# microsoft/mgl

Hardware: AMD Instinct MI355X
Metric: GCUPS (+ aligned reads/s) for 150 bp short-read batch (higher is better)
Workload: dtype int16; 1 GPU; BASELINE.json configs[1]: 10000000 Illumina-style 150 bp reads x 256-base reference windows, affine-gap SW, full matrix, GATK params (200,-150,260,11), SOFTCLIP, scores+offset+CIGAR for every pair; pairs_total=10000000, pairs_per_gpu=10000000, target_len=256, query_len=150, input=ascii, parallelism=1 GPU, steps_in_flight=1

## Files before the change

### mgl_amd/csrc/sw_capi.cpp

```cpp
#include "../../include/mgl_sw.h"

#include <hip/hip_runtime.h>

#include <algorithm>
#include <chrono>
#include <cstdint>
#include <cstdio>
#include <functional>
#include <future>
#include <cstring>
#include <mutex>
#include <string>
#include <vector>

#include "sw_ctx_access.h"
#include "sw_device.h"

using namespace mgl_sw_dev;

static_assert(sizeof(mgl_sw_score) == sizeof(Score), "mgl_sw_score layout");

namespace {

constexpr int64_t kDefaultWorkspace = 4ll << 30;
// ... 828 lines not shown
                HIP_TRY(ctx, hipEventSynchronize(ctx->srt_done[k & 3]));
                RegroupArgs ra;
                (void)sort_chunk(first, count, (int)(k & 3), &ra);
                rg.d_t_start = ra.t_start;
                rg.d_q_start = ra.q_start;
                rg.d_dest = ra.dest;
                rg.d_t_len = ra.t_len;
                rg.d_q_len = ra.q_len;
                rg.n_grouped = ctx->pin_total[2 * (k & 3)];
                rg.n_lane = ctx->pin_total[2 * (k & 3) + 1];
                if (rg.n_grouped < 0 || rg.n_grouped > count || (rg.n_grouped & 7) || rg.n_lane < 0 || rg.n_lane > rg.n_grouped || (rg.n_lane & 127))
                    return fail(ctx, MGL_SW_ERR_DEVICE, "sorting a chunk by geometry failed");
                if (!hooks) {
                    const int src = sort_until(k + 2);
                    if (src != MGL_SW_OK) return src;
                }
                sort_more = hooks != nullptr;
            }
            const SeqSet ts{tset.data, rg.d_t_start, rg.d_t_len, max_tl, tset.packed2}, qs{qset.data, rg.d_q_start, rg.d_q_len, max_ql, qset.packed2};
            const int64_t ng = rg.n_grouped;
            const char *const lgm = getenv("MGL_SW_DEBUG_LANE_GROUP_MIN");
            const int64_t lane_group_min = lgm ? (int64_t)atoll(lgm) : kLaneGroupMinPairs;
            const int64_t nl = lane_group && rg.n_lane >= std::max<int64_t>(lane_group_min, 128) ? rg.n_lane : 0;
            uint32_t *const tb16 = tb_base + (size_t)std::min<int64_t>(nl / 128, lane_slots) * (size_t)lane_group_stride;
            lane_pairs_last = nl;
            if (nl > 0) parts.push_back(Part{true, false, 0, nl, ts, qs, tb_base, lane_group_stride, rec_base, rg.d_dest, 32, 4, max_ql, false});
            if (P.group_regions) {
                uint32_t *const area16 = tb_base + (size_t)lane_slots * (size_t)lane_group_stride, *const area32 = area16 + (size_t)(P.left_area / 2 / 4);
                const int64_t cap16 = std::max<int64_t>(8, P.left_area / 2 / P.left_pair16 / 8 * 8), cap32 = std::max<int64_t>(4, P.left_area / 2 / P.left_pair32 / 4 * 4);
                for (int64_t f = nl; f < ng; f += cap16)
                    parts.push_back(Part{false, true, f, std::min(cap16, ng - f), ts, qs, area16, stride_words, rec_base + f, rg.d_dest, 16, wpb16, sps_for(max_ql), f + cap16 < ng});
                for (int64_t f = ng; f < count; f += cap32)
                    parts.push_back(Part{false, false, f, std::min(cap32, count - f), ts, qs, area32, stride32_words, rec_base + f, rg.d_dest, 16,
                                         pick_waves_per_block(sps32, 16), sps32, f + cap32 < count});
            } else {
                if (ng > nl) parts.push_back(Part{false, true, nl, ng - nl, ts, qs, tb16, stride_words, rec_base + nl, rg.d_dest, 16, wpb16, sps_for(max_ql), false});
                if (count > ng)
                    parts.push_back(Part{false, false, ng, count - ng, ts, qs, tb16 + (size_t)((ng - nl) / 2) * (size_t)stride_words, stride32_words,
                                         rec_base + ng, rg.d_dest, 16, pick_waves_per_block(sps32, 16), sps32, false});
            }
        }
        const int n_parts = (int)parts.size();
        const char *const sre = getenv("MGL_SW_DEBUG_SIDE_RESERVE");
        const int64_t side_reserve = sre ? atoll(sre) : kSideReserve;
        const bool side = P.group_regions && side_reserve > 0;
        std::vector<DpArgs> das((size_t)n_parts);
        std::vector<TbArgs> tas((size_t)n_parts);
        int64_t n_blocks = 0;
        for (int i = 0; i < n_parts; ++i) {
            const Part &pt = parts[i];
            DpArgs &da = das[i];
            da.t = pt.t;
            da.q = pt.q;
            da.first = pt.first;
            da.count = pt.count;
            da.match = match;
            da.mismatch = mismatch;
            da.gopen = gopen;
            da.gext = gext;
            da.strategy = strategy;
            da.sps_cap = pt.sps_cap;
            da.uni_tl = max_tl;
            da.uni_ql = max_ql;
            da.tb = pt.tb;
            da.tb_stride_words = pt.stride;
            da.rec = pt.rec;
            da.scratch = pt.lane ? static_cast<unsigned char *>(ctx->bnd[h].p) : (use_scratch || coop_waves || strip16) ? static_cast<unsigned char *>(ctx->scratch.p) : nullptr;
            da.diag = nullptr;
            da.matrix = d_matrix;
            da.code = d_code;
            da.matrix_lds_offset = 0;
            da.score_only = score_only ? 1 : 0;
            da.grouped = pt.lane && auto_group ? 1 : 0;
            da.strip_k = strip16 ? strip_k : 0;
            da.strip_passes = strip16 ? strip_passes : 0;
            {
                const char *const sce = getenv("MGL_SW_DEBUG_STRIP_CODES");
                da.strip_codes = strip16 && strip_k > 0 && !(sce && atoi(sce) == 0) && strip16_lds_bytes_codes(max_ql, strip_waves) <= 64 * 1024 ? 1 : 0;
            }
            da.fold_k = P.fold.k;
            da.fold_bm = P.fold.bm;
            da.fold_bx = P.fold.bx;
            da.lane_slots = 0;
            da.tile_ctr = nullptr;
            da.grid_fault = nullptr;
            da.gate = nullptr;
            da.gate_dev = nullptr;
            da.gate_failed = nullptr;
            da.gate_timeout_ticks = 0;
            if (pt.lane && (lane_ck || da.grouped)) {
                da.lane_slots = (int)std::min<int64_t>(lane_slots - (side && n_parts > 1 ? std::min<int64_t>(side_reserve, lane_slots / 2) : 0), (pt.count + 127) / 128);
                if (ctx->cur_gate && !hooks) {
                    da.gate = ctx->cur_gate;
                    da.gate_dev = ctx->cur_gate_dev;
                    da.gate_failed = reinterpret_cast<int32_t *>(const_cast<int64_t *>(ctx->cur_gate) + 1);
                    da.gate_timeout_ticks = 100000000u;
                    if (const char *const gte = getenv("MGL_SW_DEBUG_GATE_TIMEOUT_TICKS")) da.gate_timeout_ticks = (unsigned)atoll(gte);
                }
                if ((pt.count + 127) / 128 > da.lane_slots) {
                    da.tile_ctr = static_cast<unsigned *>(ctx->tile_ctr.p) + (size_t)(ctx->tile_seq++ % kTileCounters) * kTileCounterWords;
                    void *fault_dev = nullptr;
                    HIP_TRY(ctx, hipHostGetDevicePointer(&fault_dev, ctx->pin_fault, 0));
                    da.grid_fault = static_cast<int32_t *>(fault_dev);
                }
            }
            const int per_block = pt.lane ? pt.wpb * 128 : pt.packed ? pt.wpb * 8 : strip16 ? 1 : pt.wpb * (64 / pt.rows);
            if (i == 0) n_blocks = da.lane_slots > 0 ? da.lane_slots : (pt.count + per_block - 1) / per_block;
            if (ctx->profiling == 2 && i == 0) {
                HIP_TRY(ctx, ctx->diag.reserve((size_t)n_blocks * 16));
                da.diag = static_cast<unsigned long long *>(ctx->diag.p);
            }
            TbArgs &ta = tas[i];
            ta.t = pt.t;
            ta.q = pt.q;
            ta.first = pt.first;
            ta.count = pt.count;
            ta.strategy = strategy;
            ta.tb = pt.tb;
            ta.tb_stride_words = pt.stride;
            ta.packed16 = pt.lane ? 2 : pt.packed ? 1 : strip16 ? (strip_k ? 6 : 4) : coop16 ? 3 : 0;
            ta.match = match;
            ta.mismatch = mismatch;
            ta.gopen = gopen;
            ta.gext = gext;
            ta.strip_rows = pt.rows;
            ta.strip_k = strip16 ? strip_k : 0;
            ta.rows_per_stripe = pt.rows;
            ta.uni_ql = max_ql;
            ta.rec = pt.rec;
            ta.offset = d_offset;
            ta.score = d_score;
            ta.cigar = d_cigar;
            ta.cigar_stride = cigar_stride;
            ta.binary_cigar = binary_cigar ? 1 : 0;
            ta.cigar_len = d_cigar_len;
            ta.status = d_status;
            ta.status_any = hooks ? hooks->d_status_any : ctx->direct_status_any;
            ta.dest = pt.dest;
            const char *const colds = getenv("MGL_SW_DEBUG_COALESCED_OUT");
            ta.coalesced_out = pt.lane && (lane_ck || da.grouped) && !(colds && atoi(colds) == 0) && lane_ck_coalesced_ok(ta) ? 1 : 0;
        }

        hipEvent_t pe[4] = {nullptr, nullptr, nullptr, nullptr};
        if (ctx->profiling) {
            while ((int)ctx->pool.size() < ctx->pool_used + 4) {
                hipEvent_t e = nullptr;
                HIP_TRY(ctx, hipEventCreate(&e));
                ctx->pool.push_back(e);
            }
            for (int i = 0; i < 4; ++i) pe[i] = ctx->pool[(size_t)ctx->pool_used + i];
            ctx->pool_used += 4;
            ctx->diag_blocks = n_blocks;
        }
        hipStream_t tb_stream = overlap ? ctx->aux : fs;
        if ((overlap || side) && tb_pending[h]) HIP_TRY(ctx, hipStreamWaitEvent(fs, ctx->tb_done[h], 0));
        if (side && n_parts > 1) {
            if (k == 0 && ctx->ws_idle_set) HIP_TRY(ctx, hipStreamWaitEvent(ctx->aux, ctx->ws_idle, 0));
            if (side_grid_pending[h]) HIP_TRY(ctx, hipStreamWaitEvent(ctx->aux, ctx->fill_done[h], 0));
            for (int i = 0; i < n_parts; ++i) {
                const Part &pt = parts[i];
                if (pt.lane) continue;
                HIP_TRY(ctx, pt.packed ? launch_dp16(das[i], pt.wpb, ctx->aux) : launch_dp(das[i], pt.wpb, pt.rows, ctx->aux));
                HIP_TRY(ctx, launch_traceback(tas[i], ctx->aux));
            }
            HIP_TRY(ctx, hipEventRecord(ctx->tb_done[h], ctx->aux));
            tb_pending[h] = true;
// ... 1967 lines not shown
```

### mgl_amd/csrc/sw_device.h

```cpp
#ifndef MGL_SW_DEVICE_H
#define MGL_SW_DEVICE_H

#include <hip/hip_runtime.h>
#include <stddef.h>
#include <stdint.h>

namespace mgl_sw_dev {

constexpr int NEG_INF = -0x40000000;
constexpr int OS_SOFTCLIP = 1, OS_INDEL = 2, OS_LEAD_ID = 4, OS_IGNORE = 8;
constexpr int ERR_CIGAR_OVERFLOW = 2;
constexpr int ERR_DEVICE = 4;
constexpr int MATRIX_DIM = 32;

struct Score {
    int32_t mqe, mqe_t, max, max_t, max_q, seg_length;
};

struct DpRecord {
    int32_t mqe, mqe_t, max, max_t, max_q, seg;
    int32_t g_tail;
    int32_t sps;
};

struct SeqSet {
    const uint8_t *data;
    const int64_t *off;
    const int32_t *len;
    int uni_len;
    int packed2;
    __host__ __device__ inline int length(int64_t p) const
    {
        if (len) return len[p];
        return packed2 ? uni_len : (int)(off[p + 1] - off[p]);
    }
    __device__ inline int at(int64_t start, int k) const
    {
        const int64_t pos = start + k;
        if (packed2) return (data[pos >> 2] >> (2 * (int)(pos & 3))) & 3;
        return data[pos];
    }
};

struct DpArgs {
    SeqSet t, q;
    int64_t first;
    int64_t count;
    int match, mismatch, gopen, gext, strategy;
    int sps_cap;
    int uni_tl, uni_ql;
    uint32_t *tb;
    int64_t tb_stride_words;
    DpRecord *rec;
    unsigned char *scratch;
    unsigned long long *diag;
    const int8_t *matrix;
    const uint8_t *code;
    int matrix_lds_offset;
    int score_only;
    int grouped;
    int strip_k;
    int strip_passes;
    int strip_codes;
    int lane_slots;
    unsigned *tile_ctr;
    int32_t *grid_fault;
    const int64_t *gate;
    int64_t *gate_dev;
    int32_t *gate_failed;
    unsigned gate_timeout_ticks;
    const int32_t *tile_order;
    const int64_t *slot_off;
    int fold_k, fold_bm, fold_bx;
};

struct TbArgs {
    SeqSet t, q;
    int64_t first, count;
    int strategy;
    const uint32_t *tb;
    int64_t tb_stride_words;
    int packed16;
    int rows_per_stripe;
    int uni_ql;
    const DpRecord *rec;
    int32_t *offset;
    Score *score;
    char *cigar;
    int cigar_stride;
    int binary_cigar;
    int32_t *cigar_len;
    int32_t *status;
    int32_t *status_any;
    int match, mismatch, gopen, gext;
    int strip_rows, strip_k;
    const int64_t *dest;
    int coalesced_out;
};

__host__ __device__ inline int sps_for_rows(int ql, int rows) { return (ql + rows + 3) & ~3; }
__host__ __device__ inline int sps_for(int ql) { return sps_for_rows(ql, 16); }
__host__ __device__ inline int stripes_for(int tl) { return (tl + 15) >> 4; }
__host__ __device__ inline int dp_ring_entries(int sps_cap, int rows) { return sps_cap + rows + 4; }
__host__ __device__ inline int dp_qcopy_bytes(int sps_cap, int rows) { return sps_cap + rows + 16; }
__host__ __device__ inline int64_t tb_words_for(int tl, int sps, int rows)
{
    return ((((int64_t)(tl + rows - 1) / rows) * sps + 31) >> 5) * rows * 4;
}

__host__ __device__ inline int dp16_base(int tl, int ql, int match, int gext)
{
    return 32767 - match * (tl < ql ? tl : ql) - gext * (tl + ql);
}
__host__ __device__ inline int dp16_period(int ql) { return (ql + 1 + 3) & ~3; }
__host__ __device__ inline int dp16_chained_stripes(int tl, int ql)
{
    if (dp16_period(ql) < 32) return 0;
    const int n = stripes_for(tl);
    return (tl & 15) == 0 ? n : n - 1;
}
__host__ __device__ inline int64_t dp16_total_steps(int tl, int ql)
{
    const int n = stripes_for(tl), nc = dp16_chained_stripes(tl, ql);
    return (nc ? (int64_t)nc * dp16_period(ql) + 16 : 0) + (int64_t)(n - nc) * sps_for(ql);
}
__host__ __device__ inline int64_t tb_words16_for(int tl, int ql) { return ((dp16_total_steps(tl, ql) + 7) >> 3) * 32; }
__host__ __device__ inline int64_t tb_words16_bound(int tl, int ql) { return (((int64_t)stripes_for(tl) * sps_for(ql) + 16 + 7) >> 3) * 32; }

__host__ __device__ inline int lane_strips(int tl, int rows) { return (tl + rows - 1) / rows; }
__host__ __device__ inline int64_t lane_tb_words(int tl, int ql, int rows) { return (int64_t)lane_strips(tl, rows) * ql * (rows / 16) * 64 * 4; }
__host__ __device__ inline int64_t lane_bnd_entries(int ql) { return (int64_t)(ql + 1) * 64; }
__host__ __device__ inline int64_t lane_scratch_bytes(int tl, int ql, int rows)
{
    return lane_bnd_entries(ql) * 8 + ((int64_t)((ql + 3) / 4) + (int64_t)lane_strips(tl, rows) * (rows / 4)) * 2 * 64 * 4;
}

__host__ __device__ inline int coop_sps_for(int ql) { return (ql + 64 + 31) & ~31; }
__host__ __device__ inline int coop16_sps_for(int ql) { return (ql + 129 + 31) & ~31; }
__host__ __device__ inline int64_t tb_words_coop16(int tl, int ql) { return (int64_t)((tl + 127) >> 7) * (coop16_sps_for(ql) >> 4) * 64 * 4; }
__host__ __device__ inline int coop_query_bytes(int sps_cap) { return (sps_cap + 192 + 15) & ~15; }
__host__ __device__ inline int coop_wrap_cols(int sps_cap) { return sps_cap + 192; }

constexpr int LANE_CK_COLS = 32;
__host__ __device__ inline int lane_ck_blocks(int ql) { return (ql + LANE_CK_COLS - 1) / LANE_CK_COLS; }
__host__ __device__ inline int64_t lane_ck_words(int tl, int ql)
{
    const int64_t strips = lane_strips(tl, 32);
    return ((strips + 1) * (ql + 1) * 2 + strips * ql * 2 + strips * (lane_ck_blocks(ql) - 1) * 64 + (int64_t)LANE_CK_COLS * 4) * 64;
}
__host__ __device__ inline int64_t lane_ck_scratch_bytes(int tl, int ql) { return ((int64_t)((ql + 3) / 4) + (int64_t)lane_strips(tl, 32) * 8) * 2 * 64 * 4; }
constexpr int LANE_CK_OUT_STRIDE_MAX = 64;
constexpr int LANE_CK_OUT_LDS_BYTES = 128 * (LANE_CK_OUT_STRIDE_MAX + 24 + 12);
__host__ inline bool lane_ck_coalesced_ok(const TbArgs &a)
{
    auto al = [](const void *p) { return (reinterpret_cast<uintptr_t>(p) & 15u) == 0; };
    return !a.dest && !a.binary_cigar && a.cigar_stride >= 4 && a.cigar_stride <= LANE_CK_OUT_STRIDE_MAX && (a.cigar_stride & 3) == 0 && al(a.cigar) && al(a.offset) &&
           al(a.score) && al(a.cigar_len) && al(a.status) && (a.first & 127) == 0;
}
constexpr int LANE_CK_WAVES_PER_CU = 8;
__host__ __device__ inline int64_t lane_ck_region_bytes(int tl, int ql) { return lane_ck_words(tl, ql) * 4 + lane_ck_scratch_bytes(tl, ql); }
__host__ __device__ inline int64_t lane_ck_slots(int64_t pairs, int n_cus, int64_t bytes, int tl, int ql)
{
    const int64_t tiles = (pairs + 127) / 128, chip = (int64_t)n_cus * LANE_CK_WAVES_PER_CU, fit = bytes / lane_ck_region_bytes(tl, ql);
    const int64_t s = tiles < chip ? tiles : chip;
    return s < fit ? s : fit;
}

int64_t dp_group_bytes(int sps_cap, int rows);
int dp_lds_bytes(int sps_cap, int waves_per_block, int rows);
int dp16_lds_bytes(int sps, int waves_per_block);
bool dp16_range_ok(int tl, int ql, int match, int mismatch, int gopen, int gext, int strategy);
struct DiagFold {
    int k, bm, bx;
};
__host__ __device__ inline int ctz16(unsigned x)
{
    int s = 0;
    while (!(x & 1u)) x >>= 1, ++s;
    return s;
}
__host__ __device__ inline unsigned inv_odd16(unsigned o)
{
    unsigned x = o;
    for (int i = 0; i < 3; ++i) x *= 2u - o * x;
    return x & 0xffffu;
}
__host__ __device__ inline int fold_byte(unsigned k, unsigned v)
{
    const int s = ctz16(k);
    if (v & ((1u << s) - 1u)) return -1;
    const unsigned b = ((v >> s) * inv_odd16(k >> s)) & ((0x10000u >> s) - 1u);
    return b <= 255u ? (int)b : -1;
}
__host__ __device__ inline DiagFold diag_fold(int match, int mismatch, int gext)
{
    const unsigned a = (unsigned)(match + 2 * gext) & 0xffffu, x = (unsigned)(mismatch + 2 * gext) & 0xffffu;
    const unsigned p = a ? a : x;
    DiagFold d{0, 0, 0};
    if (!p) return DiagFold{1, 0, 0};
    for (unsigned b = 1; b < 256u; ++b) {
        const int u = ctz16(b);
        if (p & ((1u << u) - 1u)) continue;
        const unsigned period = 0x10000u >> u;
        for (unsigned k = ((p >> u) * inv_odd16(b >> u)) & (period - 1u); k < 0x10000u && (d.k == 0 || k < (unsigned)d.k); k += period) {
            if (k == 0) continue;
            const int bm = fold_byte(k, a), bx = fold_byte(k, x);
            if (bm >= 0 && bx >= 0) {
                d = DiagFold{(int)k, bm, bx};
                break;
            }
        }
    }
    return d;
}
hipError_t launch_dp16(const DpArgs &a, int waves_per_block, hipStream_t stream);
bool lane16_supported(const SeqSet &t, const SeqSet &q);
bool lane16_ck_supported(const SeqSet &t, const SeqSet &q);
struct TbArgs;
hipError_t launch_dp16_lane(const DpArgs &a, const TbArgs &walk, int rows, hipStream_t stream);
bool lane16_matrix_params_ok(int smin, int smax, int gopen, int gext);
int lane16_matrix_lds_bytes(int max_tl);
hipError_t launch_dp16_lane_matrix(const DpArgs &a, const TbArgs &walk, hipStream_t stream);
__host__ __device__ inline int64_t lane16_matrix_tb_bytes(int tl, int ql, bool score_only) { return score_only ? 0 : lane_tb_words(tl, ql, 32) * 4; }
__host__ __device__ inline int64_t lane16_matrix_region_bytes(int tl, int ql, bool score_only) { return (lane16_matrix_tb_bytes(tl, ql, score_only) + lane_scratch_bytes(tl, ql, 32) + 255) / 256 * 256; }
hipError_t launch_tile_geometry(const SeqSet &t, const SeqSet &q, int64_t first, int64_t count, int32_t *out, hipStream_t stream);
hipError_t launch_dp16_lane_ck(const DpArgs &a, const TbArgs &walk, hipStream_t stream);
hipError_t launch_dp(const DpArgs &a, int waves_per_block, int rows, hipStream_t stream);
int coop_lds_bytes(int sps_cap, int waves_per_block);
hipError_t launch_dp_coop(const DpArgs &a, int waves_per_block, hipStream_t stream);
bool coop16_possible(int match, int mismatch, int gopen, int gext);
bool coop16_worthwhile(int match, int mismatch, int gopen, int gext);
int coop16_lds_bytes(int sps_cap, int waves_per_block);
constexpr int STRIP_CPS = 4;
__host__ __device__ inline int strip16_groups(int ql) { return (ql + STRIP_CPS - 1) / STRIP_CPS; }
__host__ __device__ inline int strip16_steps(int ql, int waves) { return strip16_groups(ql) + 2 * 64 * waves - 1; }
// ... 94 lines not shown
```

### mgl_amd/csrc/sw_dp16_lane_ck.hip

```cpp
#include <hip/hip_runtime.h>
#include <stdint.h>
#include <stdio.h>
#include <stdlib.h>
#include <string.h>

#include "sw_device.h"
#include "sw_lane_cell.h"
#include "sw_traceback.h"

#ifndef MGL_CK_ABLATE
#define MGL_CK_ABLATE 0
#endif
#if (MGL_CK_ABLATE != 0 || defined(MGL_CK_PHASES) || defined(MGL_CK_TRACE)) && !defined(MGL_VARIANT_BUILD)
#error "MGL_CK_ABLATE / MGL_CK_PHASES are measurement builds (scripts/build_variant.sh defines MGL_VARIANT_BUILD): never the shipped library"
#endif

#ifdef MGL_CK_PHASES
__device__ unsigned long long mgl_ck_phase_ticks[16];
#define CK_PHASE(k)                                                                                    \
    do {                                                                                               \
        const unsigned long long now_ = __builtin_amdgcn_s_memtime();                                  \
        if (lane == 0) atomicAdd(&mgl_ck_phase_ticks[k], now_ - phase_t0);                             \
        phase_t0 = __builtin_amdgcn_s_memtime();                                                       \
    } while (0)
// ... 489 lines not shown
    {
        const unsigned ia = (unsigned)((((sA >> 1) * (g.nb - 1) + max(bA - 1, 0)) * 64 + (sA & 1) * 2 * RB) * 64) + wm.lane;
        const unsigned ib = (unsigned)((((sB >> 1) * (g.nb - 1) + max(bB - 1, 0)) * 64 + (sB & 1) * 2 * RB) * 64) + wm.lane;
        unsigned v[2 * RB];
#pragma unroll
        for (int x = 0; x < 2 * RB; ++x) v[x] = 0u;
        if (needA && bA > 0) {
#pragma unroll
            for (int x = 0; x < 2 * RB; ++x) v[x] = WaveMem::at32<unsigned>(wm.cku, 4u * (ia + (unsigned)(x * 64)));
        }
#pragma unroll
        for (int r = 0; r < RB; ++r) {
            const int rowA = sA * RB + r + 1;
            const int fa_ = border(rowA, g.gopen, g.gext, g.indel) + rowA * g.gext + g.base;
            h[r] = bA > 0 ? v[2 * r] : (unsigned)fa_;
            f[r] = bA > 0 ? v[2 * r + 1] : (unsigned)(fa_ - (g.gopen - g.gext));
        }
#pragma unroll
        for (int x = 0; x < 2 * RB; ++x) v[x] = 0u;
        if (needB && bB > 0) {
#pragma unroll
            for (int x = 0; x < 2 * RB; ++x) v[x] = WaveMem::at32<unsigned>(wm.cku, 4u * (ib + (unsigned)(x * 64)));
        }
#pragma unroll
        for (int r = 0; r < RB; ++r) {
            const int rowB = sB * RB + r + 1;
            const int fb_ = border(rowB, g.gopen, g.gext, g.indel) + rowB * g.gext + g.base;
            const unsigned hb = bB > 0 ? v[2 * r] : (unsigned)fb_ << 16, gb = bB > 0 ? v[2 * r + 1] : (unsigned)(fb_ - (g.gopen - g.gext)) << 16;
            h[r] = lo_hi(h[r], hb);
            f[r] = lo_hi(f[r], gb);
        }
    }
    unsigned hd;
    {
        unsigned a0 = 0u, b0 = 0u;
        if (needA) a0 = wm.row16(sA, g.ql, CK * bA).x;
        if (needB) b0 = wm.row16(sB, g.ql, CK * bB).x;
        if (sA & 1) {
            const int row = sA * RB;
            const int v = border(row, g.gopen, g.gext, g.indel) + row * g.gext + g.base;
            a0 = bA > 0 ? a0 : (unsigned)v;
        }
        if (sB & 1) {
            const int row = sB * RB;
            const int v = border(row, g.gopen, g.gext, g.indel) + row * g.gext + g.base;
            b0 = bB > 0 ? b0 : (unsigned)v << 16;
        }
        hd = lo_hi(a0, b0);
    }
    const int qmax = ((g.ql + 3) >> 2) - 1;
#pragma unroll 1
    for (int gg = 0; gg < groups; ++gg) {
        uint2 va[8], vb[8];
#pragma unroll
        for (int u = 0; u < 8; ++u) va[u] = vb[u] = make_uint2(0u, 0u);
        if (needA) {
#pragma unroll
            for (int u = 0; u < 8; ++u) va[u] = wm.row16(sA, g.ql, min(CK * bA + 8 * gg + u + 1, g.ql));
        }
        if (needB) {
#pragma unroll
            for (int u = 0; u < 8; ++u) vb[u] = wm.row16(sB, g.ql, min(CK * bB + 8 * gg + u + 1, g.ql));
        }
        unsigned qa[2], qb[2];
#pragma unroll
        for (int u = 0; u < 2; ++u) {
            qa[u] = wm.qblock(min(bA * (CK / 4) + 2 * gg + u, qmax), 0);
            qb[u] = wm.qblock(min(bB * (CK / 4) + 2 * gg + u, qmax), 1);
        }
#pragma unroll
        for (int u = 0; u < 8; ++u) {
            unsigned e = lo_hi(va[u].y, vb[u].y);
            uint4 *const out = wm.blk + (size_t)(8 * gg + u) * 64;
            if (CODES)
                column<RB, false, false, CODES>(h, f, t, code_table((qa[u >> 2] >> (8 * (u & 3))) & 0xffu, c.bm, c.bx), hd, e, c, out, nullptr,
                                                code_table((qb[u >> 2] >> (8 * (u & 3))) & 0xffu, c.bm, c.bx));
            else
                column<RB, false, false, false>(h, f, t, __builtin_amdgcn_perm(qb[u >> 2], qa[u >> 2], 0x0c040c00u + 0x00010001u * (u & 3)), hd, e, c, out);
            hd = lo_hi(va[u].x, vb[u].x);
        }
    }
}

typedef uint32_t dwords4 __attribute__((ext_vector_type(4), aligned(4)));
__device__ __forceinline__ void seq_words4(const SeqWords &s, const int k0, unsigned (&w)[4])
{
    if (k0 + 3 <= s.kmax) {
        const dwords4 v = *reinterpret_cast<const dwords4 *>(s.base + k0);
        w[0] = v.x;
        w[1] = v.y;
        w[2] = v.z;
        w[3] = v.w;
    } else {
#pragma unroll
        for (int u = 0; u < 4; ++u) w[u] = s.word(k0 + u);
    }
}
template <bool CODES, bool QUERY>
__device__ __forceinline__ unsigned stage_ascii(const uint8_t *seqA, const uint8_t *seqB, const int len, const int nblocks, unsigned *dst)
{
    SeqWords sa, sb;
    sa.init(seqA, len);
    sb.init(seqB, len);
    unsigned bad = 0;
    for (int cb = 0; cb < nblocks; cb += 16) {
        unsigned wa[20], wb[20];
#pragma unroll
        for (int u = 0; u < 4; ++u) {
            unsigned xa[4], xb[4];
            seq_words4(sa, cb + 4 * u, xa);
            seq_words4(sb, cb + 4 * u, xb);
#pragma unroll
            for (int x = 0; x < 4; ++x) {
                wa[4 * u + x] = xa[x];
                wb[4 * u + x] = xb[x];
            }
        }
        wa[16] = sa.word(cb + 16);
        wb[16] = sb.word(cb + 16);
#pragma unroll
        for (int u = 0; u < 16; ++u) {
            if (cb + u < nblocks) {
                unsigned va = __builtin_amdgcn_alignbyte(wa[u + 1], wa[u], sa.shift), vb = __builtin_amdgcn_alignbyte(wb[u + 1], wb[u], sb.shift);
                if (CODES) {
                    unsigned da, db;
                    va = ascii_codes(va, da);
                    vb = ascii_codes(vb, db);
                    if (QUERY) {
                        const unsigned na = nonzero_bytes(da), nb = nonzero_bytes(db);
                        va = ((va << 3) & ~((na >> 2) - (na >> 7))) | (na >> 2);
                        vb = ((vb << 3) & ~((nb >> 2) - (nb >> 7))) | (nb >> 2);
                    } else {
                        const int nv = len - 4 * (cb + u);
                        const unsigned keep = nv >= 4 ? 0xffffffffu : nv <= 0 ? 0u : (1u << (8 * nv)) - 1u;
                        bad |= (da | db) & keep;
                    }
                }
                dst[(size_t)(2 * (cb + u)) * 64] = va;
                dst[(size_t)(2 * (cb + u) + 1) * 64] = vb;
            }
        }
    }
    return bad;
}

struct Seq2Words {
    const uint32_t *base;
    unsigned shift;
    int kmax;
    __device__ __forceinline__ void init(const uint8_t *data, int64_t start, int len)
    {
        const uintptr_t a = reinterpret_cast<uintptr_t>(data) + (uintptr_t)(start >> 2), e = reinterpret_cast<uintptr_t>(data) + (uintptr_t)((start + len - 1) >> 2);
        base = reinterpret_cast<const uint32_t *>(a & ~(uintptr_t)3);
        shift = (unsigned)(a & 3) * 8u + 2u * (unsigned)(start & 3);
        kmax = (int)(((e & ~(uintptr_t)3) - (a & ~(uintptr_t)3)) >> 2);
    }
    __device__ __forceinline__ unsigned word(int k) const { return base[k < kmax ? k : kmax]; }
};
template <bool QUERY>
__device__ __forceinline__ void stage_2bit(const uint8_t *data, const int64_t startA, const int64_t startB, const int len, const int nblocks, unsigned *dst)
{
    Seq2Words sa, sb;
    sa.init(data, startA, len);
    sb.init(data, startB, len);
    for (int cb = 0; cb < nblocks; cb += 16) {
        unsigned wa[5], wb[5];
#pragma unroll
        for (int u = 0; u < 5; ++u) {
            wa[u] = sa.word((cb >> 2) + u);
            wb[u] = sb.word((cb >> 2) + u);
        }
#pragma unroll
        for (int u = 0; u < 4; ++u) {
            const unsigned va = __builtin_amdgcn_alignbit(wa[u + 1], wa[u], sa.shift), vb = __builtin_amdgcn_alignbit(wb[u + 1], wb[u], sb.shift);
#pragma unroll
            for (int x = 0; x < 4; ++x) {
                const int blk = cb + 4 * u + x;
                if (blk < nblocks) {
                    const unsigned ca = spread_2bit((va >> (8 * x)) & 0xffu), cb2 = spread_2bit((vb >> (8 * x)) & 0xffu);
                    dst[(size_t)(2 * blk) * 64] = QUERY ? ca << 3 : ca;
                    dst[(size_t)(2 * blk + 1) * 64] = QUERY ? cb2 << 3 : cb2;
                }
            }
        }
    }
}

__device__ __forceinline__ void lds_to_global(void *dst, const unsigned char *src, const int bytes, const int lane)
{
    const int whole = bytes & ~15;
    for (int k = lane * 16; k < whole; k += 1024) *reinterpret_cast<uint4 *>(static_cast<unsigned char *>(dst) + k) = *reinterpret_cast<const uint4 *>(src + k);
    for (int k = whole + lane * 4; k < bytes; k += 256) *reinterpret_cast<unsigned *>(static_cast<unsigned char *>(dst) + k) = *reinterpret_cast<const unsigned *>(src + k);
}

template <bool VIA_LDS, bool FOLD>
__device__ __forceinline__ void sw_dp16_lane_ck_tile(const DpArgs &a, const TbArgs &walk_in, const int64_t gw, const int64_t slot, const int lane, unsigned char *out_lds, const bool first)
{
    const int64_t n_ls = (a.count + 1) >> 1;
#ifdef MGL_CK_PHASES
    unsigned long long phase_t0 = __builtin_amdgcn_s_memtime();
#endif
    const int64_t ls = gw * 64 + lane;
    const bool lvalid = ls < n_ls;
    const int64_t slotA = lvalid ? 2 * ls : a.count - 1;
    const bool validB = lvalid && (2 * ls + 1 < a.count);
    const int64_t slotB = validB ? 2 * ls + 1 : slotA;

    const bool grouped = a.grouped != 0;
    const int tl = grouped ? __builtin_amdgcn_readfirstlane(a.t.length(a.first + gw * 128)) : a.uni_tl;
    const int ql = grouped ? __builtin_amdgcn_readfirstlane(a.q.length(a.first + gw * 128)) : a.uni_ql;
    const int match = a.match, gopen = a.gopen, gext = a.gext;
    const bool indel = (a.strategy & (OS_INDEL | OS_LEAD_ID)) != 0;
    const int base = dp16_base(tl, ql, match, gext);
    LaneConsts c;
    c.delta = pack2(a.mismatch - match, a.mismatch - match);
    c.one = pack2(1, 1);
    c.o_e = pack2(gopen - gext, gopen - gext);
    c.k2 = pack2(match + 2 * gext, match + 2 * gext);
    asm volatile("" : "+v"(c.delta), "+v"(c.one), "+v"(c.o_e), "+v"(c.k2));
#pragma unroll
    for (int u = 0; u < 4; ++u) {
        c.k12[u] = 0x02020202u << (2 * u);
        c.k34[u] = 0x01010101u << (2 * u);
        asm volatile("" : "+s"(c.k12[u]), "+s"(c.k34[u]));
    }
    c.kf = pack2(a.fold_k, a.fold_k);
    c.bm = FOLD ? (unsigned)a.fold_bm : 0u;
    c.bx = FOLD ? (unsigned)a.fold_bx : 1u;
    if (FOLD) asm volatile("" : "+s"(c.kf));
    constexpr int CM = FOLD ? CMP_FOLD : CMP_CODES;

    const int strips = lane_strips(tl, R), nb = lane_ck_blocks(ql);
    unsigned *const qst = reinterpret_cast<unsigned *>(a.scratch + (size_t)slot * (size_t)lane_ck_scratch_bytes(a.uni_tl, a.uni_ql)) + lane;
    unsigned *const tst = qst + (size_t)((ql + 3) >> 2) * 128;
    WaveMem wm;
    {
        uint2 *const region = reinterpret_cast<uint2 *>(a.tb + (size_t)slot * (size_t)a.tb_stride_words);
        wm.bnd = region + lane;
        wm.mid = wm.bnd + (size_t)(strips + 1) * (ql + 1) * 64;
        wm.ck = reinterpret_cast<unsigned *>(region + ((size_t)(strips + 1) * (ql + 1) + (size_t)strips * ql) * 64) + lane;
        wm.blk = reinterpret_cast<uint4 *>(reinterpret_cast<unsigned *>(region) + ((size_t)(strips + 1) * (ql + 1) * 2 + (size_t)strips * ql * 2 + (size_t)strips * (nb - 1) * 64) * 64) + lane;
        wm.rows = region;
        wm.mid_off = (unsigned)((strips + 1) * (ql + 1) * 64);
        wm.cku = reinterpret_cast<const unsigned *>(region + ((size_t)(strips + 1) * (ql + 1) + (size_t)strips * ql) * 64);
        wm.blku = reinterpret_cast<const uint32_t *>(region) + ((size_t)(strips + 1) * (ql + 1) * 2 + (size_t)strips * ql * 2 + (size_t)strips * (nb - 1) * 64) * 64;
        wm.seq = reinterpret_cast<const unsigned *>(a.scratch + (size_t)slot * (size_t)lane_ck_scratch_bytes(a.uni_tl, a.uni_ql));
        wm.t_off = (unsigned)(((ql + 3) >> 2) * 128);
        wm.lane = (unsigned)lane;
    }
    bool codes;
    {
        const int64_t pA = a.first + slotA, pB = a.first + slotB;
        const int qblocks = (ql + 3) >> 2, tblocks = strips * (R / 4);
        if (a.t.packed2) {
            stage_2bit<false>(a.t.data, a.t.off[pA], a.t.off[pB], tl, tblocks, tst);
            stage_2bit<true>(a.q.data, a.q.off[pA], a.q.off[pB], ql, qblocks, qst);
            codes = true;
        } else {
            const unsigned bad = stage_ascii<true, false>(a.t.data + a.t.off[pA], a.t.data + a.t.off[pB], tl, tblocks, tst);
            codes = __builtin_amdgcn_ballot_w64(bad != 0u) == 0;
            if (codes) {
                stage_ascii<true, true>(a.q.data + a.q.off[pA], a.q.data + a.q.off[pB], ql, qblocks, qst);
            } else {
                stage_ascii<false, false>(a.t.data + a.t.off[pA], a.t.data + a.t.off[pB], tl, tblocks, tst);
                stage_ascii<false, true>(a.q.data + a.q.off[pA], a.q.data + a.q.off[pB], ql, qblocks, qst);
            }
        }
        if (grouped || first) {
            for (int j = 0; j <= ql; ++j) {
                const int hb0 = border(j, gopen, gext, indel) + j * gext + base;
                const unsigned hp = pack2(hb0, hb0);
                wm.bnd[(size_t)j * 64] = make_uint2(hp, pk_sub(hp, c.o_e));
            }
            for (int k = 1; k <= strips; ++k) {
                const int hb0 = border(k * R, gopen, gext, indel) + k * R * gext + base;
                wm.bnd[(size_t)k * (ql + 1) * 64] = make_uint2(pack2(hb0, hb0), 0u);
            }
        }
    }
// ... 75 lines not shown
        if (half ? validB : lvalid) a.rec[half ? slotB : slotA] = r;
    }

    CK_PHASE(2);
    const int64_t pA = a.first + slotA, pB = a.first + slotB;
    constexpr bool via_lds = VIA_LDS;
    TbArgs walk = walk_in;
    unsigned char *const l_score = out_lds + 128 * LANE_CK_OUT_STRIDE_MAX, *const l_off = l_score + 128 * 24, *const l_len = l_off + 512, *const l_status = l_len + 512;
    if (via_lds) {
        walk.cigar = reinterpret_cast<char *>(out_lds);
        walk.score = walk_in.score ? reinterpret_cast<Score *>(l_score) : nullptr;
        walk.offset = reinterpret_cast<int32_t *>(l_off);
        walk.cigar_len = walk_in.cigar_len ? reinterpret_cast<int32_t *>(l_len) : nullptr;
        walk.status = walk_in.status ? reinterpret_cast<int32_t *>(l_status) : nullptr;
    }
    const int64_t oA = via_lds ? 2 * lane : walk.dest ? walk.dest[pA] : pA, oB = via_lds ? 2 * lane + 1 : walk.dest ? walk.dest[pB] : pB;
    PathWalk wa, wb;
    wa.start(walk, rec[0], oA, tl, ql, lvalid, cornerA);
    wb.start(walk, rec[1], oB, tl, ql, validB, cornerB);
    BlockGeom geom;
    geom.ql = ql;
    geom.nb = nb;
    geom.match = match;
    geom.mismatch = a.mismatch;
    geom.gopen = gopen;
    geom.gext = gext;
    geom.base = base;
    geom.indel = indel;
    geom.codes = codes;
    const bool by_score = !(MGL_CK_ABLATE & 8);
    const int tblocks = strips * (R / 4), qblocks = (ql + 3) >> 2;
    while (!(MGL_CK_ABLATE & 1) && __builtin_amdgcn_ballot_w64(!wa.done || !wb.done) != 0) {
        if (by_score) {
            for (;;) {
                unsigned ta[17], qa[17], tb[17], qb[17], ga[PathWalk::VB], gb[PathWalk::VB];
                if (wa.can_verify()) {
                    wa.win64_load(wm, 0, tblocks, qblocks, ta, qa);
                    wa.grid_load(wm, ql, ga);
                }
                if (wb.can_verify()) {
                    wb.win64_load(wm, 1, tblocks, qblocks, tb, qb);
                    wb.grid_load(wm, ql, gb);
                }
                const bool ma = wa.verify_apply(ta, qa, ga, 0, geom), mb = wb.verify_apply(tb, qb, gb, 1, geom);
#ifdef MGL_CK_PHASES
                if (lane == 0) atomicAdd(&mgl_ck_phase_ticks[12], 1ull);
#endif
                if (!__builtin_amdgcn_ballot_w64(ma || mb)) break;
            }
            {
                const int ea = wa.edge_len(), eb = wb.edge_len();
                if (__builtin_amdgcn_ballot_w64((ea | eb) != 0)) {
                    unsigned ta[5], qa[5], tb[5], qb[5], ha = 0u, hb = 0u;
                    if (ea) {
                        wa.win_load(wm, 0, tblocks, qblocks, ta, qa);
                        ha = wa.edge_load(wm, nb, ea);
                    }
                    if (eb) {
                        wb.win_load(wm, 1, tblocks, qblocks, tb, qb);
                        hb = wb.edge_load(wm, nb, eb);
                    }
                    const bool xa = wa.edge_apply(ha, ta, qa, ea, 0, geom), xb = wb.edge_apply(hb, tb, qb, eb, 1, geom);
#ifdef MGL_CK_PHASES
                    const unsigned long long took_ = __popcll(__builtin_amdgcn_ballot_w64(xa)) + __popcll(__builtin_amdgcn_ballot_w64(xb));
                    const unsigned long long tried_ = __popcll(__builtin_amdgcn_ballot_w64(ea != 0)) + __popcll(__builtin_amdgcn_ballot_w64(eb != 0));
                    if (lane == 0) {
                        atomicAdd(&mgl_ck_phase_ticks[10], took_);
                        atomicAdd(&mgl_ck_phase_ticks[11], tried_ - took_);
                    }
#else
                    (void)xa;
                    (void)xb;
#endif
                }
            }
            CK_PHASE(3);
            if (__builtin_amdgcn_ballot_w64(!wa.done || !wb.done) == 0) break;
        }
        const int kA = max(wa.pi - 1, 0) >> 4, bA = max(wa.pj - 1, 0) / CK, kB = max(wb.pi - 1, 0) >> 4, bB = max(wb.pj - 1, 0) / CK;
        int reach = max(!wa.done ? (max(wa.pj - 1, 0) % CK) + 1 : 0, !wb.done ? (max(wb.pj - 1, 0) % CK) + 1 : 0);
#pragma unroll
        for (int m = 32; m >= 1; m >>= 1) reach = max(reach, __shfl_xor(reach, m));
        const int groups = __builtin_amdgcn_readfirstlane((reach + 7) >> 3);
        if (codes)
            ck_block<CM>(kA, bA, kB, bB, !wa.done, !wb.done, geom, wm, c, groups);
        else
            ck_block<CMP_BYTES>(kA, bA, kB, bB, !wa.done, !wb.done, geom, wm, c, groups);
        asm volatile("s_waitcnt vmcnt(0)" ::: "memory");
        CK_PHASE(4);
#ifdef MGL_CK_PHASES
        if (lane == 0) atomicAdd(&mgl_ck_phase_ticks[8], 1ull);
#endif
        for (;;) {
            const bool la = wa.can_load(kA, bA), lb = wb.can_load(kB, bB);
            unsigned fa[PathWalk::LOOK], fb[PathWalk::LOOK], ta[5], qa[5], tb[5], qb[5];
            if (la) {
                wa.load(wm, fa);
                if (wa.mode == 0) wa.win_load(wm, 0, tblocks, qblocks, ta, qa);
            }
            if (lb) {
                wb.load(wm, fb);
                if (wb.mode == 0) wb.win_load(wm, 1, tblocks, qblocks, tb, qb);
            }
            const bool ga = wa.apply(fa, ta, qa, 0, kA, bA, geom), gb = wb.apply(fb, tb, qb, 1, kB, bB, geom);
            if (!__builtin_amdgcn_ballot_w64(ga || gb)) break;
        }
        wa.stuck = wb.stuck = false;
        CK_PHASE(5);
    }
    CK_PHASE(6);
    if (lvalid) wa.finish(walk, a.rec + slotA, oA);
    if (validB) wb.finish(walk, a.rec + slotB, oB);
    if (via_lds) {
        __builtin_amdgcn_fence(__ATOMIC_RELEASE, "workgroup");
        __builtin_amdgcn_wave_barrier();
        __builtin_amdgcn_fence(__ATOMIC_ACQUIRE, "workgroup");
        const int64_t p0 = a.first + gw * 128;
        const int np = (int)min((int64_t)128, a.count - gw * 128);
        lds_to_global(walk_in.cigar + (size_t)p0 * walk_in.cigar_stride, out_lds, np * walk_in.cigar_stride, lane);
        if (walk_in.score) lds_to_global(walk_in.score + p0, l_score, np * 24, lane);
        lds_to_global(walk_in.offset + p0, l_off, np * 4, lane);
        if (walk_in.cigar_len) lds_to_global(walk_in.cigar_len + p0, l_len, np * 4, lane);
        if (walk_in.status) lds_to_global(walk_in.status + p0, l_status, np * 4, lane);
        __builtin_amdgcn_wave_barrier();
    }
    CK_PHASE(7);
#ifdef MGL_CK_PHASES
    if (lane == 0) atomicAdd(&mgl_ck_phase_ticks[9], 1ull);
#endif
}

}

template <bool VIA_LDS, bool FOLD>
__device__ __forceinline__ void lane_ck_grid(const DpArgs &a, const TbArgs &walk, unsigned char *out_lds)
{
    const int lane = threadIdx.x & 63;
    const int64_t tiles = (((a.count + 1) >> 1) + 63) >> 6, slots = gridDim.x, slot = blockIdx.x;
    unsigned long long diag_t0 = 0, diag_w0 = 0;
    if (a.diag) {
        diag_t0 = __builtin_amdgcn_s_memtime();
        diag_w0 = __builtin_amdgcn_s_memrealtime();
    }
    int64_t arrived = a.gate ? 0 : INT64_MAX;
    unsigned long long *const ctr = reinterpret_cast<unsigned long long *>(a.tile_ctr);
    for (int64_t tile = slot; tile < tiles;) {
        if (arrived < a.first + min(a.count, (tile + 2) * 128)) {
            const int64_t need = a.first + min(a.count, (tile + 2) * 128);
            int lo = 0, hi = 0, flags = 0;
            if (lane == 0) {
                unsigned long long since = __builtin_amdgcn_s_memrealtime();
                long long last = arrived, seen;
                for (;;) {
                    seen = (long long)__hip_atomic_load(reinterpret_cast<const unsigned long long *>(a.gate_dev), __ATOMIC_RELAXED, __HIP_MEMORY_SCOPE_AGENT);
                    if (seen >= need || seen < 0) break;
                    const unsigned long long now = __builtin_amdgcn_s_memrealtime();
                    const unsigned long long polled = __hip_atomic_load(reinterpret_cast<const unsigned long long *>(a.gate_dev) + 1, __ATOMIC_RELAXED, __HIP_MEMORY_SCOPE_AGENT);
                    if (now - polled >= 100ull) {
                        unsigned long long expect = polled;
                        if (__hip_atomic_compare_exchange_strong(reinterpret_cast<unsigned long long *>(a.gate_dev) + 1, &expect, now, __ATOMIC_RELAXED, __ATOMIC_RELAXED, __HIP_MEMORY_SCOPE_AGENT)) {
                            const long long v = (long long)__hip_atomic_load(reinterpret_cast<const unsigned long long *>(a.gate), __ATOMIC_RELAXED, __HIP_MEMORY_SCOPE_SYSTEM);
                            if (v < 0)
                                __hip_atomic_store(reinterpret_cast<long long *>(a.gate_dev), v, __ATOMIC_RELAXED, __HIP_MEMORY_SCOPE_AGENT);
                            else
                                __hip_atomic_fetch_max(reinterpret_cast<long long *>(a.gate_dev), v, __ATOMIC_RELAXED, __HIP_MEMORY_SCOPE_AGENT);
                            seen = v;
                            if (seen >= need || seen < 0) break;
                        }
                    }
                    if (seen != last) {
                        last = seen;
                        since = now;
                    } else if (now - since > (unsigned long long)a.gate_timeout_ticks) {
                        flags = 1;
                        break;
                    }
                    __builtin_amdgcn_s_sleep(32);
                }
                lo = (int)(unsigned)(unsigned long long)seen;
                hi = (int)(unsigned)((unsigned long long)seen >> 32);
            }
            lo = __builtin_amdgcn_readfirstlane(lo);
            hi = __builtin_amdgcn_readfirstlane(hi);
            flags = __builtin_amdgcn_readfirstlane(flags);
            arrived = (int64_t)((unsigned long long)(unsigned)lo | (unsigned long long)(unsigned)hi << 32);
            if (flags & 1) {
                if (lane == 0) __hip_atomic_store(a.gate_failed, 1, __ATOMIC_RELAXED, __HIP_MEMORY_SCOPE_SYSTEM);
                break;
            }
            if (arrived < 0) break;
#ifndef MGL_CK_NO_GATE_FENCE
            __builtin_amdgcn_fence(__ATOMIC_ACQUIRE, "agent");
#endif
        }
#ifdef MGL_CK_TRACE
        const unsigned long long t0 = __builtin_amdgcn_s_memrealtime();
#endif
        sw_dp16_lane_ck_tile<VIA_LDS, FOLD>(a, walk, tile, slot, lane, out_lds, tile == slot);
#ifdef MGL_CK_TRACE
        if (lane == 0 && tile < (1 << 17)) {
            unsigned hw;
            asm volatile("s_getreg_b32 %0, hwreg(HW_REG_HW_ID)" : "=s"(hw));
            unsigned xcc;
            asm volatile("s_getreg_b32 %0, hwreg(HW_REG_XCC_ID)" : "=s"(xcc));
            mgl_ck_trace[4 * tile + 0] = (unsigned long long)slot;
            mgl_ck_trace[4 * tile + 1] = (unsigned long long)hw | (unsigned long long)(xcc & 15u) << 32;
            mgl_ck_trace[4 * tile + 2] = t0;
            mgl_ck_trace[4 * tile + 3] = __builtin_amdgcn_s_memrealtime();
        }
#endif
        if (tiles <= slots) break;
        unsigned next = 0;
        if (lane == 0) {
            next = (unsigned)__hip_atomic_fetch_add(ctr, 1ull, __ATOMIC_RELAXED, __HIP_MEMORY_SCOPE_AGENT);
            if (next >= (unsigned)tiles && a.grid_fault) __hip_atomic_store(a.grid_fault, 1, __ATOMIC_RELAXED, __HIP_MEMORY_SCOPE_SYSTEM);
        }
        tile = slots + (int64_t)(unsigned)__builtin_amdgcn_readfirstlane((int)next);
    }
    if (tiles > slots && lane == 0) {
        const unsigned out = (unsigned)(__hip_atomic_fetch_add(ctr, 1ull << 32, __ATOMIC_RELAXED, __HIP_MEMORY_SCOPE_AGENT) >> 32);
        if (out == (unsigned)slots - 1u) {
            __hip_atomic_store(ctr, 0ull, __ATOMIC_RELAXED, __HIP_MEMORY_SCOPE_AGENT);
        } else if (out >= (unsigned)slots && a.grid_fault) {
            __hip_atomic_store(a.grid_fault, 1, __ATOMIC_RELAXED, __HIP_MEMORY_SCOPE_SYSTEM);
        }
    }
    if (a.diag && lane == 0) {
        a.diag[2 * slot] = __builtin_amdgcn_s_memtime() - diag_t0;
        a.diag[2 * slot + 1] = __builtin_amdgcn_s_memrealtime() - diag_w0;
    }
}

__global__ __launch_bounds__(64, 2) void sw_dp16_lane_ck_kernel(const DpArgs a, const TbArgs walk)
{
    __shared__ __attribute__((aligned(16))) unsigned char out_lds[LANE_CK_OUT_LDS_BYTES];
    lane_ck_grid<true, false>(a, walk, out_lds);
}

__global__ __launch_bounds__(64, 2) void sw_dp16_lane_ck_scatter_kernel(const DpArgs a, const TbArgs walk) { lane_ck_grid<false, false>(a, walk, nullptr); }

__global__ __launch_bounds__(64, 2) void sw_dp16_lane_ck_kernel_fold(const DpArgs a, const TbArgs walk)
{
    __shared__ __attribute__((aligned(16))) unsigned char out_lds[LANE_CK_OUT_LDS_BYTES];
    lane_ck_grid<true, true>(a, walk, out_lds);
}
__global__ __launch_bounds__(64, 2) void sw_dp16_lane_ck_scatter_kernel_fold(const DpArgs a, const TbArgs walk) { lane_ck_grid<false, true>(a, walk, nullptr); }

bool lane16_ck_supported(const SeqSet &t, const SeqSet &q) { return (t.packed2 != 0) == (q.packed2 != 0); }

hipError_t launch_dp16_lane_ck(const DpArgs &a, const TbArgs &walk, hipStream_t stream)
{
    const int64_t tiles = ((a.count + 1) / 2 + 63) / 64;
    if (a.lane_slots < 1 || (tiles > a.lane_slots && !a.tile_ctr)) return hipErrorInvalidValue;
    const dim3 grid((unsigned)(tiles < a.lane_slots ? tiles : a.lane_slots)), block(64);
    if (walk.coalesced_out)
        hipLaunchKernelGGL(a.fold_k ? sw_dp16_lane_ck_kernel_fold : sw_dp16_lane_ck_kernel, grid, block, 0, stream, a, walk);
    else
        hipLaunchKernelGGL(a.fold_k ? sw_dp16_lane_ck_scatter_kernel_fold : sw_dp16_lane_ck_scatter_kernel, grid, block, 0, stream, a, walk);
    return hipGetLastError();
}

}

#ifdef MGL_CK_TRACE
extern "C" int mgl_ck_trace_dump(const char *path)
{
    static unsigned long long h[4 << 17];
    hipDeviceSynchronize();
    if (hipMemcpyFromSymbol(h, HIP_SYMBOL(mgl_ck_trace), sizeof h) != hipSuccess) return 1;
    FILE *f = fopen(path, "wb");
    if (!f) return 2;
    fwrite(h, 1, sizeof h, f);
    fclose(f);
    memset(h, 0, sizeof h);
    hipMemcpyToSymbol(HIP_SYMBOL(mgl_ck_trace), h, sizeof h);
    return 0;
}
#endif

#ifdef MGL_CK_PHASES
extern "C" void mgl_ck_phases_dump()
{
    unsigned long long h[16] = {0};
    hipDeviceSynchronize();
    hipMemcpyFromSymbol(h, HIP_SYMBOL(mgl_ck_phase_ticks), sizeof h);
    static const char *names[8] = {"staging", "pass 1", "records", "stretches", "block flags", "walk in block", "(loop exit)", "finish"};
    unsigned long long tot = 0;
    for (int k = 0; k < 8; ++k) tot += h[k];
    for (int k = 0; k < 8; ++k) fprintf(stderr, "phase %-20s %6.2f %%  %10.1f ticks per wave\n", names[k], 100.0 * h[k] / (double)tot, (double)h[k] / (double)h[9]);
    fprintf(stderr, "waves %llu, block rounds per wave %.2f\n", h[9], (double)h[8] / (double)h[9]);
    fprintf(stderr, "edge stretches per wave: taken %.3f, tried and not adding up %.3f; verify iterations per wave %.2f\n", (double)h[10] / (double)h[9],
            (double)h[11] / (double)h[9], (double)h[12] / (double)h[9]);
    memset(h, 0, sizeof h);
    hipMemcpyToSymbol(HIP_SYMBOL(mgl_ck_phase_ticks), h, sizeof h);
}
#endif
```

Baseline: 6580 GCUPS.

## Recompute checkpoint blocks cooperatively across wave rows when few walks remain

Adds a wide block recompute path for the checkpointed traceback. When at most a threshold number of lane walks (8 by default) still need a block, 16-lane wave rows each take one pending walk and sweep the block as an anti-diagonal wavefront through DPP shifts, writing direction bits to LDS. Otherwise the existing per-lane ck_block runs. The aim is to stop paying a full-wave block recompute for only a handful of active lanes in the traceback tail, at the cost of extra LDS per block, atomics, and a serialized wavefront loop.

```diff
diff --git a/mgl_amd/csrc/sw_capi.cpp b/mgl_amd/csrc/sw_capi.cpp
--- a/mgl_amd/csrc/sw_capi.cpp
+++ b/mgl_amd/csrc/sw_capi.cpp
@@ -934,6 +934,10 @@
             da.fold_bm = P.fold.bm;
             da.fold_bx = P.fold.bx;
             da.lane_slots = 0;
+            {
+                const char *const wbe = getenv("MGL_SW_DEBUG_WIDE_BLOCKS");
+                da.wide_blocks = wbe ? std::max(0, std::min(128, atoi(wbe))) : LANE_CK_WIDE_T;
+            }
             da.tile_ctr = nullptr;
             da.grid_fault = nullptr;
             da.gate = nullptr;
diff --git a/mgl_amd/csrc/sw_device.h b/mgl_amd/csrc/sw_device.h
--- a/mgl_amd/csrc/sw_device.h
+++ b/mgl_amd/csrc/sw_device.h
@@ -72,6 +72,7 @@
     const int32_t *tile_order;
     const int64_t *slot_off;
     int fold_k, fold_bm, fold_bx;
+    int wide_blocks;
 };
 
 struct TbArgs {
@@ -151,6 +152,9 @@
 __host__ __device__ inline int64_t lane_ck_scratch_bytes(int tl, int ql) { return ((int64_t)((ql + 3) / 4) + (int64_t)lane_strips(tl, 32) * 8) * 2 * 64 * 4; }
 constexpr int LANE_CK_OUT_STRIDE_MAX = 64;
 constexpr int LANE_CK_OUT_LDS_BYTES = 128 * (LANE_CK_OUT_STRIDE_MAX + 24 + 12);
+constexpr int LANE_CK_WIDE_T = 8;
+constexpr int LANE_CK_WIDE_WALK_DWORDS = LANE_CK_COLS * 4 + LANE_CK_COLS + LANE_CK_COLS;
+constexpr int LANE_CK_WIDE_LDS_BYTES = 4 * LANE_CK_WIDE_WALK_DWORDS * 4;
 __host__ inline bool lane_ck_coalesced_ok(const TbArgs &a)
 {
     auto al = [](const void *p) { return (reinterpret_cast<uintptr_t>(p) & 15u) == 0; };
diff --git a/mgl_amd/csrc/sw_dp16_lane_ck.hip b/mgl_amd/csrc/sw_dp16_lane_ck.hip
--- a/mgl_amd/csrc/sw_dp16_lane_ck.hip
+++ b/mgl_amd/csrc/sw_dp16_lane_ck.hip
@@ -595,6 +595,139 @@
     }
 }
 
+__device__ __forceinline__ int sx16(const int x) { return (int)(short)x; }
+__device__ __forceinline__ int row_shr1(const int x) { return __builtin_amdgcn_update_dpp(0, x, 0x111, 0xf, 0xf, false); }
+__device__ __forceinline__ int ck_block_wide(const int kA, const int bA, const int kB, const int bB, const bool needA, const bool needB, const int reach,
+                                             const BlockGeom &g, const WaveMem &wm, unsigned *const lds)
+{
+    const int row = (int)(wm.lane >> 4), r = (int)(wm.lane & 15u);
+    unsigned *const my = lds + row * LANE_CK_WIDE_WALK_DWORDS;
+    unsigned long long restA = __builtin_amdgcn_ballot_w64(needA), restB = __builtin_amdgcn_ballot_w64(needB);
+    const int mt = g.match + 2 * g.gext, mm = g.mismatch + 2 * g.gext, oe = g.gopen - g.gext;
+    const int qmax = ((g.ql + 3) >> 2) - 1;
+    int passes = 0;
+    while ((restA | restB) != 0ull) {
+        ++passes;
+        int owner = 0, half = 0;
+        bool valid = false;
+#pragma unroll
+        for (int w = 0; w < 4; ++w) {
+            int o = 0, hf = 0;
+            bool v = false;
+            if (restA != 0ull) {
+                o = __builtin_ctzll(restA);
+                restA &= restA - 1ull;
+                v = true;
+            } else if (restB != 0ull) {
+                o = __builtin_ctzll(restB);
+                restB &= restB - 1ull;
+                hf = 1;
+                v = true;
+            }
+            if (row == w) {
+                owner = o;
+                half = hf;
+                valid = v;
+            }
+        }
+        const int sa = __shfl(kA, owner), sb = __shfl(kB, owner), ca = __shfl(bA, owner), cb = __shfl(bB, owner);
+        const int s = half ? sb : sa, b = half ? cb : ca;
+        const unsigned own = (unsigned)owner;
+        auto pick = [&](const unsigned v) { return half ? hi16(v) : lo16(v); };
+        const unsigned tw = WaveMem::at32<unsigned>(wm.seq, 4u * (wm.t_off + (unsigned)((2 * (s * (RB / 4) + (r >> 2)) + half) * 64) + own));
+        const unsigned tbyte = (tw >> (8 * (r & 3))) & 0xffu, tcmp = g.codes ? tbyte << 3 : tbyte;
+        int h, f;
+        {
+            const int rowi = s * RB + r + 1;
+            const int fb = border(rowi, g.gopen, g.gext, g.indel) + rowi * g.gext + g.base;
+            h = sx16(fb);
+            f = sx16(fb - oe);
+            if (b > 0) {
+                const unsigned i0 = (unsigned)((((s >> 1) * (g.nb - 1) + (b - 1)) * 64 + (s & 1) * 2 * RB + 2 * r) * 64) + own;
+                h = pick(WaveMem::at32<unsigned>(wm.cku, 4u * i0));
+                f = pick(WaveMem::at32<unsigned>(wm.cku, 4u * (i0 + 64u)));
+            }
+        }
+        auto kept = [&](const int j) {
+            const unsigned e8 = (s & 1) ? wm.mid_off + (unsigned)(((s >> 1) * g.ql + j - 1) * 64) + own : (unsigned)(((s >> 1) * (g.ql + 1) + j) * 64) + own;
+            return WaveMem::at32<uint2>(wm.rows, 8u * e8);
+        };
+        unsigned keep[2], qc[2];
+#pragma unroll
+        for (int u = 0; u < 2; ++u) {
+            const int c = r + 16 * u;
+            const uint2 v = kept(min(CK * b + c + 1, g.ql));
+            keep[u] = ((unsigned)pick(v.x) & 0xffffu) | ((unsigned)pick(v.y) << 16);
+            const unsigned qw = WaveMem::at32<unsigned>(wm.seq, 4u * ((unsigned)((2 * min((CK * b + c) >> 2, qmax) + half) * 64) + own));
+            qc[u] = (qw >> (8 * (c & 3))) & 0xffu;
+        }
+        int hd;
+        {
+            const int row0 = s * RB;
+            const int v0 = sx16(border(row0, g.gopen, g.gext, g.indel) + row0 * g.gext + g.base);
+            const unsigned e8 = (s & 1) ? wm.mid_off + (unsigned)(((s >> 1) * g.ql + max(CK * b, 1) - 1) * 64) + own : (unsigned)(((s >> 1) * (g.ql + 1) + CK * b) * 64) + own;
+            const int kv = pick(WaveMem::at32<uint2>(wm.rows, 8u * e8).x);
+            hd = ((s & 1) && b == 0) ? v0 : kv;
+        }
+        __builtin_amdgcn_fence(__ATOMIC_RELEASE, "workgroup");
+        __builtin_amdgcn_wave_barrier();
+        *reinterpret_cast<uint4 *>(my + 8 * r) = make_uint4(0u, 0u, 0u, 0u);
+        *reinterpret_cast<uint4 *>(my + 8 * r + 4) = make_uint4(0u, 0u, 0u, 0u);
+        my[4 * CK + r] = keep[0];
+        my[4 * CK + 16 + r] = keep[1];
+        my[5 * CK + r] = qc[0];
+        my[5 * CK + 16 + r] = qc[1];
+        __builtin_amdgcn_fence(__ATOMIC_RELEASE, "workgroup");
+        __builtin_amdgcn_wave_barrier();
+        __builtin_amdgcn_fence(__ATOMIC_ACQUIRE, "workgroup");
+        int eo = 0, qs = 0, dg = row_shr1(h);
+        dg = r == 0 ? hd : dg;
+        const int steps = reach + RB - 1;
+#pragma unroll 1
+        for (int t = 0; t < steps; ++t) {
+            const unsigned top = my[4 * CK + min(t, CK - 1)], tq = my[5 * CK + min(t, CK - 1)];
+            int up_h = row_shr1(h), up_e = row_shr1(eo), q = row_shr1(qs);
+            if (r == 0) {
+                up_h = lo16(top);
+                up_e = hi16(top);
+                q = (int)tq;
+            }
+            const int c = t - r;
+            const int diag = sx16(dg + ((unsigned)q != tcmp ? mm : mt));
+            const int sm = max(diag, f), hn = max(sm, up_e), open = sx16(hn - oe);
+            const unsigned bits = (sm < up_e ? 0x2u : 0u) | (f < open ? 0x1u : 0u) | (diag < f ? 0x20000u : 0u) | (up_e < open ? 0x10000u : 0u);
+            if (c >= 0 && c < reach) {
+                if (valid) __hip_atomic_fetch_or(my + 4 * c + (r >> 2), bits << (2 * (r & 3)), __ATOMIC_RELAXED, __HIP_MEMORY_SCOPE_WORKGROUP);
+                h = hn;
+                f = max(open, f);
+                eo = max(open, up_e);
+                qs = q;
+                dg = up_h;
+            }
+        }
+        __builtin_amdgcn_fence(__ATOMIC_RELEASE, "workgroup");
+        __builtin_amdgcn_wave_barrier();
+        __builtin_amdgcn_fence(__ATOMIC_ACQUIRE, "workgroup");
+        if (valid) {
+#pragma unroll
+            for (int u = 0; u < 2; ++u) {
+                const int c = 2 * r + u;
+                if (c < reach) {
+                    const uint4 v = *reinterpret_cast<const uint4 *>(my + 4 * c);
+                    unsigned char *const out = reinterpret_cast<unsigned char *>(const_cast<uint32_t *>(wm.blku)) + 4u * ((unsigned)(c * 256) + 4u * own) + (unsigned)half;
+                    const unsigned d[4] = {v.x, v.y, v.z, v.w};
+#pragma unroll
+                    for (int x = 0; x < 4; ++x) {
+                        out[4 * x] = (unsigned char)(d[x] & 0xffu);
+                        out[4 * x + 2] = (unsigned char)((d[x] >> 16) & 0xffu);
+                    }
+                }
+            }
+        }
+    }
+    return passes;
+}
+
 typedef uint32_t dwords4 __attribute__((ext_vector_type(4), aligned(4)));
 __device__ __forceinline__ void seq_words4(const SeqWords &s, const int k0, unsigned (&w)[4])
 {
@@ -707,7 +840,7 @@
 }
 
 template <bool VIA_LDS, bool FOLD>
-__device__ __forceinline__ void sw_dp16_lane_ck_tile(const DpArgs &a, const TbArgs &walk_in, const int64_t gw, const int64_t slot, const int lane, unsigned char *out_lds, const bool first)
+__device__ __forceinline__ void sw_dp16_lane_ck_tile(const DpArgs &a, const TbArgs &walk_in, const int64_t gw, const int64_t slot, const int lane, unsigned char *out_lds, unsigned *wide_lds, const bool first)
 {
     const int64_t n_ls = (a.count + 1) >> 1;
 #ifdef MGL_CK_PHASES
@@ -949,7 +1082,19 @@
 #pragma unroll
         for (int m = 32; m >= 1; m >>= 1) reach = max(reach, __shfl_xor(reach, m));
         const int groups = __builtin_amdgcn_readfirstlane((reach + 7) >> 3);
-        if (codes)
+        const int waiting = __popcll(__builtin_amdgcn_ballot_w64(!wa.done)) + __popcll(__builtin_amdgcn_ballot_w64(!wb.done));
+        if (waiting <= a.wide_blocks) {
+            const int passes_ = ck_block_wide(kA, bA, kB, bB, !wa.done, !wb.done, reach, geom, wm, wide_lds);
+#ifdef MGL_CK_PHASES
+            if (lane == 0) {
+                atomicAdd(&mgl_ck_phase_ticks[13], 1ull);
+                atomicAdd(&mgl_ck_phase_ticks[14], (unsigned long long)waiting);
+                atomicAdd(&mgl_ck_phase_ticks[15], (unsigned long long)passes_);
+            }
+#else
+            (void)passes_;
+#endif
+        } else if (codes)
             ck_block<CM>(kA, bA, kB, bB, !wa.done, !wb.done, geom, wm, c, groups);
         else
             ck_block<CMP_BYTES>(kA, bA, kB, bB, !wa.done, !wb.done, geom, wm, c, groups);
@@ -1000,7 +1145,7 @@
 }
 
 template <bool VIA_LDS, bool FOLD>
-__device__ __forceinline__ void lane_ck_grid(const DpArgs &a, const TbArgs &walk, unsigned char *out_lds)
+__device__ __forceinline__ void lane_ck_grid(const DpArgs &a, const TbArgs &walk, unsigned char *out_lds, unsigned *wide_lds)
 {
     const int lane = threadIdx.x & 63;
     const int64_t tiles = (((a.count + 1) >> 1) + 63) >> 6, slots = gridDim.x, slot = blockIdx.x;
@@ -1063,7 +1208,7 @@
 #ifdef MGL_CK_TRACE
         const unsigned long long t0 = __builtin_amdgcn_s_memrealtime();
 #endif
-        sw_dp16_lane_ck_tile<VIA_LDS, FOLD>(a, walk, tile, slot, lane, out_lds, tile == slot);
+        sw_dp16_lane_ck_tile<VIA_LDS, FOLD>(a, walk, tile, slot, lane, out_lds, wide_lds, tile == slot);
 #ifdef MGL_CK_TRACE
         if (lane == 0 && tile < (1 << 17)) {
             unsigned hw;
@@ -1101,17 +1246,27 @@
 __global__ __launch_bounds__(64, 2) void sw_dp16_lane_ck_kernel(const DpArgs a, const TbArgs walk)
 {
     __shared__ __attribute__((aligned(16))) unsigned char out_lds[LANE_CK_OUT_LDS_BYTES];
-    lane_ck_grid<true, false>(a, walk, out_lds);
-}
-
-__global__ __launch_bounds__(64, 2) void sw_dp16_lane_ck_scatter_kernel(const DpArgs a, const TbArgs walk) { lane_ck_grid<false, false>(a, walk, nullptr); }
+    __shared__ __attribute__((aligned(16))) unsigned wide_lds[LANE_CK_WIDE_LDS_BYTES / 4];
+    lane_ck_grid<true, false>(a, walk, out_lds, wide_lds);
+}
+
+__global__ __launch_bounds__(64, 2) void sw_dp16_lane_ck_scatter_kernel(const DpArgs a, const TbArgs walk)
+{
+    __shared__ __attribute__((aligned(16))) unsigned wide_lds[LANE_CK_WIDE_LDS_BYTES / 4];
+    lane_ck_grid<false, false>(a, walk, nullptr, wide_lds);
+}
 
 __global__ __launch_bounds__(64, 2) void sw_dp16_lane_ck_kernel_fold(const DpArgs a, const TbArgs walk)
 {
     __shared__ __attribute__((aligned(16))) unsigned char out_lds[LANE_CK_OUT_LDS_BYTES];
-    lane_ck_grid<true, true>(a, walk, out_lds);
-}
-__global__ __launch_bounds__(64, 2) void sw_dp16_lane_ck_scatter_kernel_fold(const DpArgs a, const TbArgs walk) { lane_ck_grid<false, true>(a, walk, nullptr); }
+    __shared__ __attribute__((aligned(16))) unsigned wide_lds[LANE_CK_WIDE_LDS_BYTES / 4];
+    lane_ck_grid<true, true>(a, walk, out_lds, wide_lds);
+}
+__global__ __launch_bounds__(64, 2) void sw_dp16_lane_ck_scatter_kernel_fold(const DpArgs a, const TbArgs walk)
+{
+    __shared__ __attribute__((aligned(16))) unsigned wide_lds[LANE_CK_WIDE_LDS_BYTES / 4];
+    lane_ck_grid<false, true>(a, walk, nullptr, wide_lds);
+}
 
 bool lane16_ck_supported(const SeqSet &t, const SeqSet &q) { return (t.packed2 != 0) == (q.packed2 != 0); }
 
@@ -1158,6 +1313,8 @@
     fprintf(stderr, "waves %llu, block rounds per wave %.2f\n", h[9], (double)h[8] / (double)h[9]);
     fprintf(stderr, "edge stretches per wave: taken %.3f, tried and not adding up %.3f; verify iterations per wave %.2f\n", (double)h[10] / (double)h[9],
             (double)h[11] / (double)h[9], (double)h[12] / (double)h[9]);
+    fprintf(stderr, "wide block rounds per wave %.2f (full rounds %.2f), walks served by them %.2f, passes %.2f\n", (double)h[13] / (double)h[9],
+            (double)(h[8] - h[13]) / (double)h[9], (double)h[14] / (double)h[9], (double)h[15] / (double)h[9]);
     memset(h, 0, sizeof h);
     hipMemcpyToSymbol(HIP_SYMBOL(mgl_ck_phase_ticks), h, sizeof h);
 }
```

Result: faster. 6660 GCUPS (median of 6 runs) (+1.2%).
